# ariana-spalter/human-robot-gym

Hardware: AMD Instinct MI355X
Metric: env steps/sec (whole node), ReachHuman+shield 4096 envs (higher is better)
Workload: dtype f64

## Files before the change

human-robot-gym_amd/csrc/hrgym_device.h:

```cpp
#pragma once
#include <hip/hip_runtime.h>
#include <stdint.h>

#include "../../include/hrgym.h"
#include "../../include/hrgym_state.h"

#define NV HRG_NV
#define NARM HRG_NARM
#ifndef HRG_BOX
#define HRG_BOX 0
#endif
#ifndef HRG_LIFT
#define HRG_LIFT 0
#endif
#ifndef HRG_HANDOVER
#define HRG_HANDOVER 0
#endif
#ifndef HRG_STACK
#define HRG_STACK 0
#endif
#ifndef HRG_HULLS
#define HRG_HULLS 0
#endif
#ifndef HRG_HAMMER
// ... 96 lines not shown
#ifdef HRG_STAMPS
static __device__ unsigned long long g_stamps[32];
static __device__ unsigned long long g_stamps_slow[34];
static __device__ unsigned long long g_slow_thresh = ~0ull;
static __device__ unsigned long long g_envcyc[16384][3];
static __device__ unsigned long long g_envacc[16384][32];
__shared__ unsigned long long g_tbeg;
__shared__ unsigned long long g_acc[32];
__shared__ unsigned long long g_t0;
#define STAMP_NOW(var) do { __builtin_amdgcn_sched_barrier(0); asm volatile("s_memtime %0\n\ts_waitcnt lgkmcnt(0)" : "=s"(var) :: "memory"); __builtin_amdgcn_sched_barrier(0); } while (0)
#define STAMP_DECL
#define STAMP_INIT(lane) do { if ((lane) < 32) g_acc[lane] = 0; unsigned long long _t; STAMP_NOW(_t); g_t0 = _t; g_tbeg = _t; __syncthreads(); } while (0)
#define STAMP(k) do { unsigned long long _t; STAMP_NOW(_t); if (threadIdx.x == 0) { g_acc[k] += _t - g_t0; g_t0 = _t; } } while (0)
#define STAMP_FLUSH(lane)
#define COUNT(k, n) do { if (threadIdx.x == 0) g_acc[k] += (n); } while (0)
#define STAMP_FINAL(lane) do { __syncthreads(); if ((lane) < 32) atomicAdd(&g_stamps[lane], g_acc[lane]); { unsigned long long _te; STAMP_NOW(_te); if (_te - g_tbeg > g_slow_thresh) { if ((lane) < 32) atomicAdd(&g_stamps_slow[lane], g_acc[lane]); if ((lane) == 32) atomicAdd(&g_stamps_slow[32], 1ull); if ((lane) == 33) atomicAdd(&g_stamps_slow[33], _te - g_tbeg); } } if ((lane) < 32 && blockIdx.x < 16384) g_envacc[blockIdx.x][lane] = g_acc[lane]; if ((lane) == 0 && blockIdx.x < 16384) { unsigned long long _t; STAMP_NOW(_t); g_envcyc[blockIdx.x][0] = g_tbeg; g_envcyc[blockIdx.x][1] = _t; unsigned _hw, _xcc; asm volatile("s_getreg_b32 %0, hwreg(HW_REG_HW_ID)\n\ts_getreg_b32 %1, hwreg(HW_REG_XCC_ID)" : "=s"(_hw), "=s"(_xcc)); g_envcyc[blockIdx.x][2] = ((unsigned long long)_xcc << 32) | _hw; } } while (0)
#else
#define STAMP_DECL
#define STAMP_INIT(lane)
#define STAMP(k)
#define STAMP_FLUSH(lane)
#define COUNT(k, n)
#define STAMP_FINAL(lane)
#endif

struct DevModel {
  hrg_model_desc m;
  double Rbase[9];
  double Rq[NV][9];
  int32_t anc_mask[NV];
  int32_t hb_maxdepth;
  double sol_K, sol_Bd;
  double rcap_hl[HRG_NRCAP], hcap_hl[HRG_NHB];
  int32_t hb_njump;
  int32_t hb_jump[4][HRG_NHB];
  int32_t phase_mask;
  hrg_path brake_full;
  double brake_T, brake_ds;
  int32_t hc_n;
  struct alignas(32) HcRec { double th, v, al; int32_t kj, pad; } hc[HRG_NHCAP_MAX];
  int32_t n_self;
  struct alignas(32) SelfRec { int32_t ij, body_j; double inv_len2, bound, r_j; } self_rec[64];
  int32_t n_chk;
  int32_t chk_i[32], chk_j[32];
  hrg_clip_table clips;
  const double* pose_tab;
  const double* hull_dev;
  double hull_cen[HRG_NHULL][3];
  unsigned long long* mpr_fallback;
  double fric_D[NV + 1], fric_lim[NV + 1];
  double eul_hd[NV], eul_rhd[2];
  int32_t eul_fingers, eul_pad;
  double rcap_mid[HRG_NRCAP][3];
};

struct Contact {
  int32_t g1, g2, b1, b2;
  double dist, n[3], pos[3];
};

#define ROW_CON0 24
#define ROW_WELD0 (ROW_CON0 + 4 * NCON_DYN)
#if HRG_HAMMER
#define HROW_NFRIC 8
#define HROW_LIM0 9
#define HROW_NLIM 25
#define HROW_EQ0 27
#define HROW_CON0 36
#define HROW_NEQ 9
#define NROW 128
#elif HRG_STACK
#define SROW_WELD0 24
#define SROW_CON0 36
#define NROW HRG_NROW_STACK
#elif HRG_BOX && (HRG_HANDOVER || HRG_LIFT)
#define NROW (ROW_WELD0 + 6)
#else
#define NROW ROW_WELD0
#endif

struct GjkLds { double y[4][3], a[4][3], b[4][3], l[4], lam[4]; int ia[4], ib[4]; };
#define HRG_HULL_MPR (HRG_HULLS && (HRG_BOX || HRG_STACK || HRG_HAMMER))
#if HRG_HULL_MPR
struct MprLds { double v[5][3], a[5][3], b[5][3]; };
#endif
struct Lds {
  hrg_env_state st;
  double kR[NV][9], kp[NV][3], Sw[NV][3], Sv[NV][3], vw[NV][3], vv[NV][3];
  double M[NV * NV];
  double bias[NV], a0[NVS], Ma0[NVS], ctrl[NV], qacc[NVS], g[NVS], d[NVS];
#if HRG_BOX
  hrg_box_state bx;
  double bR[9];
  double bMr[9];
  double hand_q[4], hand_off[3];
  int palm_hit, palm_pad;
#if HRG_HANDOVER
  double hcap_keep[HRG_NHB][6];
#endif
#endif
  double act[NV];
#if HRG_POSE_TABLE
  double hyaw[9];
#endif
  int acc_has_collision, acc_collision_type, acc_failsafe, acc_pad;
#if HRG_HAMMER
// ... 592 lines not shown
  for (int k = 0; k < NV; k++) {
    const double akk = __shfl(a, k * 9, 64);
    if (!(akk > 0)) good = false;
    const double inv = rsqrt(akk), d = akk * inv;
    const double lik = __shfl(a, i * 8 + k, 64) * inv;
    const double ljk = __shfl(a, j * 8 + k, 64) * inv;
    if (j == k) { if (i == k) a = d; else if (i > k) a = lik; }
    else if (i > k && j > k) a -= lik * ljk;
  }
  *ok = good;
  return a;
}
template <bool ZEROS = false>
DI double chain_prefix(double x, int lane) {
  double y = ZEROS || lane < NARM ? x : 0.0;
  {
#pragma clang fp contract(off)
    y += dpp_f64<0x111>(y);
  }
  y += dpp_f64<0x112>(y);
  y += dpp_f64<0x114>(y);
  return lane < NARM ? y : y + x;
}
template <bool ZEROS = false>
DI double subtree_sum(double x, int lane) {
  double y = ZEROS || lane < NV ? x : 0.0;
  {
#pragma clang fp contract(off)
    y += dpp_f64<0x101>(y);
  }
  y += dpp_f64<0x102>(y);
  y += dpp_f64<0x104>(y);
  return lane < NARM ? y : x;
}
DI double uniform_f64(double v) {
  const long long b = __double_as_longlong(v);
  const int lo = __builtin_amdgcn_readfirstlane((int)(b & 0xffffffffLL));
  const int hi = __builtin_amdgcn_readfirstlane((int)(b >> 32));
  return __longlong_as_double(((long long)hi << 32) | (unsigned int)lo);
}
typedef __attribute__((address_space(3))) double LdsF64;
DI LdsF64* lds_lane_base(double* p) {
  unsigned a = (unsigned)(size_t)(LdsF64*)p;
  asm volatile("" : "+v"(a));
  return (LdsF64*)(size_t)a;
}
template <int K>
DI double lane_value(double v) {
  const long long b = __double_as_longlong(v);
  const int lo = __builtin_amdgcn_readlane((int)(b & 0xffffffffLL), K);
  const int hi = __builtin_amdgcn_readlane((int)(b >> 32), K);
  return __longlong_as_double(((long long)hi << 32) | (unsigned int)lo);
}
DI void cull_box(const double* cap, double rr, bool has, int lane, double* lo, double* hi) {
  const int g = lane >> 4;
  const long long flip = (long long)(g & 1) << 63;
  double e1 = -1e300, e2 = -1e300;
  if (has) {
    const int a = g >> 1;
    const double p1 = __longlong_as_double(__double_as_longlong(cap[a]) ^ flip), p2 = __longlong_as_double(__double_as_longlong(cap[3 + a]) ^ flip);
    e1 = max_f64(p1, p2) + rr;
    if (g < 2) {
      const double z1 = __longlong_as_double(__double_as_longlong(cap[2]) ^ flip), z2 = __longlong_as_double(__double_as_longlong(cap[5]) ^ flip);
      e2 = max_f64(z1, z2) + rr;
    }
  }
  e1 = row16_max(e1); e2 = row16_max(e2);
  hi[0] = lane_value<0>(e1); lo[0] = -lane_value<16>(e1); hi[1] = lane_value<32>(e1); lo[1] = -lane_value<48>(e1);
  hi[2] = lane_value<0>(e2); lo[2] = -lane_value<16>(e2);
}
#define HRG_PIVOT(v, K) lane_value<(K) * 9>(v)
template <int K>
DI void inv_pivot(double& a, int i, int j, bool& good) {
  const double akk = HRG_PIVOT(a, K);
  if (!(akk > 0)) good = false;
  const double pa = 1.0 / akk;
  const double aik = __shfl(a, i * 8 + K, 64);
  const double akj = __shfl(a, K * 8 + j, 64);
  if (i == K) a = j == K ? pa : akj * pa;
  else if (j == K) a = -aik * pa;
  else a -= aik * akj * pa;
}
DI double spd_inverse1(double a, int lane, bool* ok) {
  const int i = lane >> 3, j = lane & 7;
  bool good = true;
  inv_pivot<0>(a, i, j, good); inv_pivot<1>(a, i, j, good); inv_pivot<2>(a, i, j, good); inv_pivot<3>(a, i, j, good);
  inv_pivot<4>(a, i, j, good); inv_pivot<5>(a, i, j, good); inv_pivot<6>(a, i, j, good); inv_pivot<7>(a, i, j, good);
  *ok = good;
  return a;
}
DI double spd_inverse1_6(double a, int lane, bool* ok) {
  const int i = lane >> 3, j = lane & 7;
  bool good = true;
  inv_pivot<0>(a, i, j, good); inv_pivot<1>(a, i, j, good); inv_pivot<2>(a, i, j, good); inv_pivot<3>(a, i, j, good);
  inv_pivot<4>(a, i, j, good); inv_pivot<5>(a, i, j, good);
  *ok = good;
  return a;
}
template <int K>
DI void inv_pivot4(double* a, int i, int j, bool& good) {
#pragma unroll
  for (int q = 0; q < 4; q++) inv_pivot<K>(a[q], i, j, good);
}
DI void spd_inverse4(double* a, int lane, bool* ok) {
  const int i = lane >> 3, j = lane & 7;
  bool good = true;
  inv_pivot4<0>(a, i, j, good); inv_pivot4<1>(a, i, j, good); inv_pivot4<2>(a, i, j, good); inv_pivot4<3>(a, i, j, good);
  inv_pivot4<4>(a, i, j, good); inv_pivot4<5>(a, i, j, good);
  *ok = good;
}
template <int N> struct Tiles { double t[N][N]; };
DI double lane_value_dyn(double v, int k) {
  const long long b = __double_as_longlong(v);
  const int lo = __builtin_amdgcn_readlane((int)(b & 0xffffffffLL), k);
  const int hi = __builtin_amdgcn_readlane((int)(b >> 32), k);
  return __longlong_as_double(((long long)hi << 32) | (unsigned int)lo);
}
template <int N, int A, int A0>
DI void tiles_pivots(Tiles<N>& T, int i, int j, int np, bool& good) {
#pragma unroll 1
  for (int P = 0; P < np; P++) {
    const double akk = lane_value_dyn(T.t[A][A], P * 9);
// ... 44 lines not shown
```

human-robot-gym_amd/csrc/hrgym_hip.hip:

```cpp
#include <hip/hip_runtime.h>

#include <algorithm>
#include <cmath>
#include <cstdio>
#include <cstring>
#include <cstdlib>
#include <initializer_list>
#include <limits>
#include <memory>
#include <string>
#include <vector>

#include "hrgym_kernels.h"

template <class MD>
DI void impedance(const MD& m, double x0, double* imp) {
  const double d0 = m.solimp[0], dmax = m.solimp[1], width = m.solimp[2], mid = m.solimp[3], power = m.solimp[4];
  const double x = fabs(x0) / width;
  double y;
  if (x >= 1) y = 1;
  else if (x <= 0) y = 0;
  else if (x <= mid) { const double u = x / mid; y = u * u * mid; }
  else { const double u = (1 - x) / (1 - mid); y = 1 - u * u * (1 - mid); }
  (void)power;
// ... 2178 lines not shown
  const ModelPtr dm = uniform_model(dm_);
  Lds& L = g_L;
  const auto& m = dm->m;
  hrg_env_state& s = L.st;
      s.time = s.time + m.timestep;
  eef_update(dm_);
  const int hl = dm->clips.clip_holding_hand[clip_of(dm, gid, s.episode, s.anim_index)];
  const int site = hl ? m.site_lhand : m.site_rhand;
  wave_sync();
  if (lane < 3) {
    const double mp = s.human_site[site][lane] + L.hand_off[lane];
    L.bx.mocap_pos[lane] = mp;
    if (m.task == HRG_TASK_HANDOVER_R2H) L.bx.target[lane] = mp;
  }
  if (lane < 4) L.bx.mocap_quat[lane] = L.hand_q[lane];
  wave_sync();
  robot_chain_fk(dm_, lane, false);
  robot_dynamics_terms(dm_, lane);
  for (int k = lane; k < HRG_NHB * 6; k += 64) (&L.hcap[0][0])[k] = (&L.hcap_keep[0][0])[k];
  wave_sync();
}
#endif

#ifndef HRG_FAIR
#if HRG_HANDOVER || HRG_STACK || HRG_HAMMER
#define HRG_FAIR 0
#else
#define HRG_FAIR 2
#endif
#endif
#if HRG_FAIR
#ifndef FAIR_SCOPE
#define FAIR_SCOPE __HIP_MEMORY_SCOPE_WORKGROUP
#endif
DI int fair_key() {
  unsigned hw, xcc;
  asm volatile("s_getreg_b32 %0, hwreg(HW_REG_HW_ID)\n\ts_getreg_b32 %1, hwreg(HW_REG_XCC_ID)" : "=s"(hw), "=s"(xcc));
  const unsigned wave = hw & 0xf, simd = (hw >> 4) & 3, cu = (hw >> 8) & 0xf, sh = (hw >> 12) & 1, se = (hw >> 13) & 7;
  return (int)((((((xcc & 7) * 8 + se) * 2 + sh) * 16 + cu) * 4 + simd) * 8 + (wave & 7));
}
DI void fair_publish(int* g_fair, int lane, int progress) {
  const int key = fair_key();
  if (lane == 0) __hip_atomic_store(&g_fair[key], progress + 1, __ATOMIC_RELAXED, FAIR_SCOPE);
}
DI int fair_begin(int* g_fair, int lane, int progress) {
  const int key = fair_key(), base = key & ~7;
  if (lane == 0) __hip_atomic_store(&g_fair[key], progress + 1, __ATOMIC_RELAXED, FAIR_SCOPE);
  int v = 0;
  if (lane < 8) v = __hip_atomic_load(&g_fair[base + lane], __ATOMIC_RELAXED, FAIR_SCOPE);
  return v;
}
DI void fair_apply(int lane, int progress, int v, bool busy) {
  const int me = fair_key() & 7;
  const bool other = lane < 8 && lane != me && v > 0;
  int vmin = other ? v : 0x7fffffff, vmax = other ? v : 0;
#pragma unroll
  for (int o = 4; o > 0; o >>= 1) {
    const int a = __shfl_xor(vmin, o, 64), b = __shfl_xor(vmax, o, 64);
    vmin = a < vmin ? a : vmin; vmax = b > vmax ? b : vmax;
  }
  vmin = __builtin_amdgcn_readfirstlane(vmin); vmax = __builtin_amdgcn_readfirstlane(vmax);
  const int own = progress + 1;
  int pr;
  if (vmax == 0) pr = 0;
  else {
    pr = own < vmax ? (own <= vmin ? 3 : 2)
                    : (own > vmin ? 0 : 1);
  }
  if (busy && pr < 2) pr = 2;
  pr = __builtin_amdgcn_readfirstlane(pr);
  if (pr == 3) __builtin_amdgcn_s_setprio(3);
  else if (pr == 2) __builtin_amdgcn_s_setprio(2);
  else if (pr == 1) __builtin_amdgcn_s_setprio(1);
  else __builtin_amdgcn_s_setprio(0);
}
#endif

DI int cycle_body(const DevModel* __restrict__ dm_, int lane, int e, int64_t gid, int cyc, int busy, double* dbg_r, double* dbg_h, int32_t* dbg_nh, int32_t* fair) {
  (void)fair;
  asm volatile("" : "+v"(lane));
  const ModelPtr dm = uniform_model(dm_);
  Lds& L = g_L;
  const auto& m = dm->m;
  hrg_env_state& s = L.st;
  STAMP(0);
#define FAIR_P(k) cyc
#if HRG_FAIR
  int fair_v = fair_begin(fair, lane, FAIR_P(0));
  const bool fair_busy = __builtin_amdgcn_readfirstlane((busy || !s.is_safe) ? 1 : 0) != 0;
#elif !defined(HRG_NO_PRIO)
  if (__builtin_amdgcn_readfirstlane((busy || !s.is_safe) ? 1 : 0)) __builtin_amdgcn_s_setprio(3); else __builtin_amdgcn_s_setprio(0);
#endif
  if (cyc == 0) {
    if (lane < NARM) {
      const double scale = fabs(m.act_out_max - m.act_out_min) / fabs(m.act_in_max - m.act_in_min);
      const double otr = 0.5 * (m.act_out_max + m.act_out_min), itr = 0.5 * (m.act_in_max + m.act_in_min);
      const double a = clampd(L.act[lane], m.act_in_min, m.act_in_max);
      const double g = clampd(s.qpos[lane] + ((a - itr) * scale + otr), m.qpos_limits[0][lane], m.qpos_limits[1][lane]);
      s.goal_qpos[lane] = g;
      s.new_goal_q[lane] = g;
    }
    s.new_goal = 1;
    wave_sync();
  }
#ifdef HRG_STAMPS
  const int pm = dm->phase_mask;
#else
  constexpr int pm = 0xff;
#endif
  if (pm & 1) shield_step(dm_, lane, e, dbg_r, dbg_h, dbg_nh); else robot_chain_fk(dm_, lane, false);
  STAMP(1);
#if HRG_FAIR
  fair_apply(lane, FAIR_P(0), fair_v, fair_busy);
#endif
// ... 612 lines not shown
  quatmul(mq, q1, qa);
  human_fk_lanes(dm_, lane, mp, mq, fr + 7);
  constexpr int NP = 6 * HRG_NHB + 3 * HRG_NHJ;
  double* o = out + (size_t)k * 2 * NP;
  for (int j = lane; j < 6 * HRG_NHB; j += 64) o[j] = (&L.hcap[0][0])[j];
  for (int j = lane; j < 3 * HRG_NHJ; j += 64) o[6 * HRG_NHB + j] = (&s.human_site[0][0])[j];
  wave_sync();
  human_yaw_update();
  human_pose_from_table(dm, lane, f);
  for (int j = lane; j < 6 * HRG_NHB; j += 64) o[NP + j] = (&L.hcap[0][0])[j];
  for (int j = lane; j < 3 * HRG_NHJ; j += 64) o[NP + 6 * HRG_NHB + j] = (&s.human_site[0][0])[j];
}

__global__ __launch_bounds__(64) void hrg_wave_helpers_kernel(const double* __restrict__ in, unsigned long long mask, double* __restrict__ out) {
  const int lane = hrg_lane();
  const double x = in[lane];
  for (int k = 0; k < HRG_WAVE_NOUT; k++) out[64 * k + lane] = __builtin_nan("");
  if ((mask >> lane) & 1) {
    double* o = out + lane;
    o[64 * 0] = wave_sum(x);
    o[64 * 1] = row8_sum(x);
    o[64 * 2] = row16_max(x);
    o[64 * 3] = wave_max(x);
    o[64 * 4] = chain_prefix(x, lane);
    o[64 * 5] = subtree_sum(x, lane);
    o[64 * 6] = fsqrt(x);
    o[64 * 7] = dpp_f64<0xB1>(x);
    o[64 * 8] = dpp_f64<0x4E>(x);
    o[64 * 9] = dpp_f64<0x141>(x);
    o[64 * 10] = dpp_f64<0x140>(x);
    o[64 * 11] = dpp_f64<0x111>(x);
    o[64 * 12] = dpp_f64<0x112>(x);
    o[64 * 13] = dpp_f64<0x114>(x);
    o[64 * 14] = dpp_f64<0x101>(x);
    o[64 * 15] = dpp_f64<0x102>(x);
    o[64 * 16] = dpp_f64<0x104>(x);
    o[64 * 17] = dpp_f64_rows<0x142, 0xa>(x);
    o[64 * 18] = dpp_f64_rows<0x143, 0xc>(x);
    o[64 * 19] = __builtin_amdgcn_rsq(x);
    o[64 * 20] = chain_prefix<true>(lane < NARM ? x : 0.0, lane);
    o[64 * 21] = subtree_sum<true>(lane < NV ? x : 0.0, lane);
  }
}

__global__ __launch_bounds__(64) void hrg_cull_box_kernel(const double* __restrict__ in, int n, double* __restrict__ out) {
  const int lane = hrg_lane();
  const bool has = (lane & 15) < n;
  const int c = has ? lane & 15 : 0;
  double lo[3], hi[3];
  cull_box(in + 7 * c, in[7 * c + 6], has, lane, lo, hi);
  if (lane == 0) for (int a = 0; a < 3; a++) { out[a] = lo[a]; out[3 + a] = hi[a]; }
}

struct ModelConstants { double fric_D, fric_lim, fric_imp, eul_hd, eul_rhd, rcap_mid; int eul_fingers; };
static_assert(3 * HRG_NRCAP <= 64, "one lane per coordinate of a capsule's mid point");
DI ModelConstants model_constants(ModelPtr dm, int lane, double x0) {
  const auto& m = dm->m;
  ModelConstants c = {0, 0, 0, 0, 0, 0, 0};
  if (lane <= NV) {
    const bool nail = lane == NV;
    const int r = nail ? 0 : lane;
    const double floss = nail ? m.hm_nail_frictionloss : m.jnt_frictionloss[r], diag = nail ? m.hm_nail_invweight : m.dof_invweight0[r];
    if (floss > 0 && diag > 0) {
      c.fric_D = row_D(m, x0, diag, &c.fric_imp);
      c.fric_lim = floss / c.fric_D;
    }
  }
  {
    const double h = m.timestep;
    const double hd6 = h * m.jnt_damping[NARM], hd7 = h * m.jnt_damping[NARM + 1];
    const bool fingers = hd6 > 0 && hd7 > 0;
    c.eul_fingers = fingers;
    if (lane < NV) c.eul_hd = h * m.jnt_damping[lane];
    if (lane < 2) c.eul_rhd = fingers ? 1.0 / (lane ? hd7 : hd6) : 0.0;
  }
  if (lane < 3 * HRG_NRCAP) {
    const int cc = lane / 3, a = lane - 3 * cc;
    c.rcap_mid = 0.5 * (m.rcap_p1[cc][a] + m.rcap_p2[cc][a]);
  }
  return c;
}
__global__ __launch_bounds__(64) void hrg_model_constants_kernel(DevModel* __restrict__ dmw) {
  const ModelPtr dm = uniform_model(dmw);
  const int lane = hrg_lane();
  const ModelConstants c = model_constants(dm, lane, 0.0);
  if (lane <= NV) { dmw->fric_D[lane] = c.fric_D; dmw->fric_lim[lane] = c.fric_lim; }
  if (lane < NV) dmw->eul_hd[lane] = c.eul_hd;
  if (lane < 2) dmw->eul_rhd[lane] = c.eul_rhd;
  if (lane == 0) dmw->eul_fingers = c.eul_fingers;
  if (lane < 3 * HRG_NRCAP) (&dmw->rcap_mid[0][0])[lane] = c.rcap_mid;
}
__global__ __launch_bounds__(64) void hrg_model_constants_tap_kernel(const DevModel* __restrict__ dm_, double x0, double* __restrict__ out) {
  const ModelPtr dm = uniform_model(dm_);
  const int lane = hrg_lane();
  const ModelConstants c = model_constants(dm, lane, x0);
  double* st = out, *re = out + HRG_MC_DIM;
  if (lane <= NV) {
    const bool fr = dm_->fric_D[lane] != 0;
    st[HRG_MC_FRIC_D + lane] = dm_->fric_D[lane]; re[HRG_MC_FRIC_D + lane] = c.fric_D;
    st[HRG_MC_FRIC_LIM + lane] = dm_->fric_lim[lane]; re[HRG_MC_FRIC_LIM + lane] = c.fric_lim;
    st[HRG_MC_FRIC_IMP + lane] = fr ? dm->m.solimp[0] : 0.0; re[HRG_MC_FRIC_IMP + lane] = c.fric_imp;
  }
  if (lane < NV) { st[HRG_MC_EUL_HD + lane] = dm_->eul_hd[lane]; re[HRG_MC_EUL_HD + lane] = c.eul_hd; }
  if (lane < 2) { st[HRG_MC_EUL_RHD + lane] = dm_->eul_rhd[lane]; re[HRG_MC_EUL_RHD + lane] = c.eul_rhd; }
  if (lane == 0) { st[HRG_MC_EUL_FINGERS] = dm_->eul_fingers; re[HRG_MC_EUL_FINGERS] = c.eul_fingers; }
  if (lane < 3 * HRG_NRCAP) { st[HRG_MC_RCAP_MID + lane] = (&dm_->rcap_mid[0][0])[lane]; re[HRG_MC_RCAP_MID + lane] = c.rcap_mid; }
}
#endif

__global__ __launch_bounds__(64) void HRG_SYM(hrg_chain_fk_kernel)(const DevModel* __restrict__ dm_, const double* __restrict__ q, int n, int shield_on, double* __restrict__ out) {
  const int lane = hrg_lane(), k = (int)blockIdx.x;
  if (k >= n) return;
  Lds& L = g_L;
  const double* qk = q + (size_t)k * 3 * NARM;
  if (lane < NARM) { L.cq[lane] = qk[lane]; L.qe[lane] = qk[NARM + lane]; }
  if (lane < NV) L.st.qpos[lane] = lane < NARM ? qk[2 * NARM + lane] : 0.0;
  wave_sync();
  robot_chain_fk(dm_, lane, shield_on != 0);
  double* o = out + (size_t)k * HRG_CFK_DIM;
  for (int j = lane; j < 9 * NV; j += 64) o[HRG_CFK_KR + j] = (&L.kR[0][0])[j];
  if (lane < 3 * NV) o[HRG_CFK_KP + lane] = (&L.kp[0][0])[lane];
  for (int j = lane; j < 2 * HRG_NSHIELD_RCAP * 6; j += 64) o[HRG_CFK_SCAP + j] = shield_on ? (&L.scap[0][0][0])[j] : 0.0;
}

__global__ __launch_bounds__(64) void HRG_SYM(hrg_self_pairs_kernel)(const DevModel* __restrict__ dm_, const double* __restrict__ q, int n, double* __restrict__ out) {
  const int lane = hrg_lane(), k = (int)blockIdx.x;
  if (k >= n) return;
  const ModelPtr dm = uniform_model(dm_);
  Lds& L = g_L;
  if (lane < NV) L.st.qpos[lane] = lane < NARM ? q[(size_t)k * NARM + lane] : 0.0;
  wave_sync();
  robot_chain_fk(dm_, lane, false);
  wave_sync();
  robot_capsules_world(dm, lane);
  wave_sync();
  double* o = out + (size_t)k * HRG_SP_DIM;
  if (lane < 6 * HRG_NRCAP) o[HRG_SP_CAPS + lane] = (&L.rcapw[0][0])[lane];
  const bool valid = lane < dm->n_self;
  const SelfPair sp = self_pair(dm, valid ? lane : 0);
  const bool near = valid && self_near(sp);
  double* op = o + HRG_SP_PAIRS + HRG_SP_PDIM * lane;
  for (int a = 0; a < HRG_SP_PDIM; a++) op[a] = 0.0;
  if (valid) { op[0] = sp.i; op[1] = sp.j; op[2] = near ? 1.0 : 0.0; }
// ... 168 lines not shown
```

human-robot-gym_amd/csrc/hrgym_host_batch.h:

```cpp

struct TaskTraits;
struct hrg_batch {
  int device = 0;
  int32_t n_envs = 0;
  int64_t env_id0 = 0;
  DeviceMem mem;
  DevModel* d_model = nullptr;
  double* d_frames = nullptr;
  double* d_pose = nullptr;
  size_t pose_bytes = 0;
  double* d_hull = nullptr;
  bool hulls = false;
  unsigned long long* d_mpr_fallback = nullptr;
  hrg_env_state* d_states = nullptr;
  double* d_rcaps = nullptr;
  double* d_hcaps = nullptr;
  int32_t* d_nh = nullptr;
  float* d_scratch_obs = nullptr;
  hrg_box_state* d_boxes = nullptr;
  hrg_stack_state* d_stacks = nullptr;
  hrg_hammer_state* d_hammers = nullptr;
  int32_t* d_order = nullptr;
  int32_t parity = 0;
  const TaskTraits* traits = nullptr;
// ... 141 lines not shown
    if (desc->scap_body[c] != (c < NARM ? c : NARM - 1)) return fail(HRG_ERR_INVALID, "shield capsule c must sit on link c (gripper on link 6)");
  if (desc->n_bodypart > HRG_NBODYPART_MAX || desc->n_extremity > HRG_NEXTREMITY_MAX) return fail(HRG_ERR_INVALID, "too many body parts");
  const TaskTraits* const t = task_traits(desc->task);
  if (!t) return fail(HRG_ERR_UNSUPPORTED, "unknown task");
  if (desc->task == HRG_TASK_STACKING) {
    if (!(desc->box_inertia[0] == desc->box_inertia[1] && desc->box_inertia[1] == desc->box_inertia[2]))
      return fail(HRG_ERR_UNSUPPORTED, "CollaborativeStackingCart: the HIP stepper stacks cubes (object_full_size with three equal edges)");
    for (int c = 0; c < clips->n_clips; c++) {
      const int32_t* kf = clips->clip_stack_keyframes[c];
      if (!(kf[0] >= 0 && kf[0] <= kf[1] && kf[1] <= kf[2] && kf[2] <= kf[3] && kf[3] <= kf[4] && clips->clip_n_loop[c] >= 0 && clips->clip_n_loop[c] <= HRG_MAX_LOOP &&
            clips->clip_n_loop2[c] >= 0 && clips->clip_n_loop2[c] <= HRG_MAX_LOOP))
        return fail(HRG_ERR_INVALID, "CollaborativeStackingCart: every clip needs five ascending keyframes and at most 4 loop sines per waiting phase in its info");
    }
  }
  if (desc->task == HRG_TASK_LIFTING && !(desc->min_balance > -1 && desc->min_balance < 1)) return fail(HRG_ERR_INVALID, "CollaborativeLiftingCart: min_balance must lie in (-1, 1)");
  if (HRG_IS_HANDOVER(desc->task))
    for (int c = 0; c < clips->n_clips; c++)
      if (!(clips->clip_n_loop2[c] >= 0 && clips->clip_n_loop2[c] <= HRG_MAX_LOOP)) return fail(HRG_ERR_INVALID, "HumanRobotHandoverCart: at most 4 loop sines per stage");
  if (desc->task == HRG_TASK_INSPECTION || HRG_IS_HANDOVER(desc->task))
    for (int c = 0; c < clips->n_clips; c++)
      if (!(clips->clip_n_loop[c] >= 0 && clips->clip_n_loop[c] <= HRG_MAX_LOOP && clips->clip_keyframes[c][0] >= 0 && clips->clip_keyframes[c][0] <= clips->clip_keyframes[c][1]))
        return fail(HRG_ERR_INVALID, "HumanObjectInspectionCart: every clip needs keyframes (k0 <= k1) and at most 4 loop sines in its info");
  if (desc->ik_enabled && !(desc->ik_max_iter >= 1 && desc->ik_max_iter <= 1000 && desc->ik_damping > 0 && desc->ik_action_limit > 0 && desc->ik_residual_threshold >= 0))
    return fail(HRG_ERR_INVALID, "ik: need 1 <= max_iter <= 1000, damping > 0, action_limit > 0, residual_threshold >= 0");
  if (desc->task == HRG_TASK_HAMMERING) {
    if (!(desc->hm_board_mass > 0 && desc->hm_hammer_mass > 0 && desc->hm_nail_mass > 0 && desc->hm_nail_range > 0 && desc->hm_nail_invweight > 0 && desc->n_obj_placements > 0 &&
          desc->hm_board_inertia[0] > 0 && desc->hm_board_inertia[1] > 0 && desc->hm_board_inertia[2] > 0 && desc->hm_hammer_inertia[0] > 0 && desc->hm_hammer_inertia[1] > 0 &&
          desc->hm_hammer_inertia[2] > 0))
      return fail(HRG_ERR_INVALID, "CollaborativeHammeringCart needs positive board / hammer / nail masses and inertias, a nail range and n_obj_placements > 0");
    for (int c = 0; c < clips->n_clips; c++)
      if (!(clips->clip_keyframes[c][0] >= 0 && clips->clip_keyframes[c][0] <= clips->clip_keyframes[c][1] && clips->clip_n_loop[c] >= 0 && clips->clip_n_loop[c] <= HRG_MAX_LOOP))
        return fail(HRG_ERR_INVALID, "CollaborativeHammeringCart: every clip needs two ascending keyframes and at most 4 loop sines in its info");
  } else
  if (t->objs != HRG_OBJ_NONE && !(desc->box_half[0] > 0 && desc->box_half[1] > 0 && desc->box_half[2] > 0 && desc->box_mass > 0 && desc->box_inertia[0] > 0 && desc->box_inertia[1] > 0 &&
                                     desc->box_inertia[2] > 0 && desc->box_inertia_mean > 0 && desc->box_invweight_rot > 0 && desc->n_targets > 0 && desc->n_obj_placements > 0))
    return fail(HRG_ERR_INVALID, "PickPlaceHumanCart needs box_half, box_mass, box_inertia, n_targets, n_obj_placements > 0");
  int maxd = 0;
  for (int i = 0; i < HRG_NHB; i++) maxd = desc->hb_depth[i] > maxd ? desc->hb_depth[i] : maxd;
  if (maxd + 1 > 16) return fail(HRG_ERR_INVALID, "human tree deeper than 15");
  int n_in_pos = 0;
  for (int k = 0; k < desc->n_bodypart; k++) {
    if (desc->bp_joint[k][0] < 0 || desc->bp_joint[k][0] >= HRG_NHJ || desc->bp_joint[k][1] < 0 || desc->bp_joint[k][1] >= HRG_NHJ) return fail(HRG_ERR_INVALID, "body part joint outside the human's sites");
    n_in_pos += desc->bp_in_pos[k] ? 1 : 0;
  }
  for (int k = 0; k < desc->n_extremity; k++)
    if (desc->ext_joint[k] < 0 || desc->ext_joint[k] >= HRG_NHJ) return fail(HRG_ERR_INVALID, "extremity joint outside the human's sites");
  if (2 * desc->n_bodypart + desc->n_extremity + n_in_pos > HRG_NHCAP_MAX) return fail(HRG_ERR_INVALID, "more than 64 human reach capsules");
  int64_t tot = 0;
  for (int c = 0; c < clips->n_clips; c++) {
    if (clips->clip_len[c] < 1 || clips->clip_offset[c] != tot) return fail(HRG_ERR_INVALID, "clip table must be densely packed");
    tot += clips->clip_len[c];
  }
  if (tot != clips->total_frames) return fail(HRG_ERR_INVALID, "clip table total_frames mismatch");
  if (desc->robot_hulls) {
    if (!g_variants.v[t->family][1].step)
      return fail(HRG_ERR_UNSUPPORTED, "robot_hulls: no hull variant of the step kernel for this task");
    if (!desc->hull_verts || desc->hull_off[0] != 0) return fail(HRG_ERR_INVALID, "robot_hulls: hull_verts / hull_off missing");
    for (int h = 0; h < HRG_NHULL; h++)
      if (!(desc->hull_off[h + 1] > desc->hull_off[h] + 3 && desc->hull_off[h + 1] <= 1000000)) return fail(HRG_ERR_INVALID, "robot_hulls: every hull needs at least four vertices");
  }
  return HRG_OK;
}

static void batch_fill_model(const hrg_model_desc* desc, const hrg_clip_table* clips, DevModel* hm) {
  memset(hm, 0, sizeof *hm);
  hm->m = *desc;
  mat_from_quat(hm->Rbase, desc->base_quat);
  for (int i = 0; i < NV; i++) {
    mat_from_quat(hm->Rq[i], desc->body_quat[i]);
    int mask = 0;
    for (int k = i; k >= 0; k = desc->body_parent[k]) mask |= 1 << k;
    hm->anc_mask[i] = mask;
  }
  int maxd = 0;
  for (int i = 0; i < HRG_NHB; i++) maxd = desc->hb_depth[i] > maxd ? desc->hb_depth[i] : maxd;
  hm->hb_maxdepth = maxd;
  {
    double tc = desc->solref[0];
    const double dr = desc->solref[1], dmax = desc->solimp[1];
    if (tc < 2 * desc->timestep) tc = 2 * desc->timestep;
    hm->sol_K = 1.0 / (dmax * dmax * tc * tc * dr * dr);
    hm->sol_Bd = 2.0 / (dmax * tc);
  }
  for (int c = 0; c < HRG_NRCAP; c++) {
    double d2 = 0;
    for (int a = 0; a < 3; a++) d2 += (desc->rcap_p2[c][a] - desc->rcap_p1[c][a]) * (desc->rcap_p2[c][a] - desc->rcap_p1[c][a]);
    hm->rcap_hl[c] = 0.5 * sqrt(d2);
  }
  for (int c = 0; c < HRG_NHB; c++) {
    double d2 = 0;
    for (int a = 0; a < 3; a++) d2 += (desc->hcap_p2[c][a] - desc->hcap_p1[c][a]) * (desc->hcap_p2[c][a] - desc->hcap_p1[c][a]);
    hm->hcap_hl[c] = 0.5 * sqrt(d2);
  }
  for (int i = 0; i < HRG_NHB; i++) hm->hb_jump[0][i] = desc->hb_parent[i];
  for (int s = 1; s < 4; s++)
    for (int i = 0; i < HRG_NHB; i++) { const int a = hm->hb_jump[s - 1][i]; hm->hb_jump[s][i] = a < 0 ? -1 : hm->hb_jump[s - 1][a]; }
  hm->hb_njump = 0;
  while ((1 << hm->hb_njump) < maxd + 1) hm->hb_njump++;
  int n = 0;
  auto hc_set = [&](int n, int kind, int j1, int j2, double th, double v, double al) { hm->hc[n].th = th; hm->hc[n].v = v; hm->hc[n].al = al; hm->hc[n].kj = kind | (j1 << 8) | (j2 << 16); hm->hc[n].pad = 0; };
  for (int k = 0; k < desc->n_bodypart; k++, n++) hc_set(n, 0, desc->bp_joint[k][0], desc->bp_joint[k][1], desc->bp_thickness[k], desc->bp_vmax[k], desc->bp_amax[k]);
  for (int k = 0; k < desc->n_bodypart; k++, n++) hc_set(n, 1, desc->bp_joint[k][0], desc->bp_joint[k][1], desc->bp_thickness[k], desc->bp_vmax[k], 0.0);
  for (int k = 0; k < desc->n_extremity; k++, n++) hc_set(n, 2, desc->ext_joint[k], desc->ext_joint[k], desc->ext_thickness[k], desc->ext_vmax[k], desc->ext_length[k]);
  for (int k = 0; k < desc->n_bodypart; k++)
    if (desc->bp_in_pos[k]) hc_set(n++, 3, desc->bp_joint[k][0], desc->bp_joint[k][1], desc->bp_thickness[k], desc->bp_vmax[k], 0.0);
  hm->hc_n = n;
  int ns = 0;
  for (int i = 0; i < HRG_NRCAP; i++)
    for (int j = i + 1; j < HRG_NRCAP; j++)
      if ((desc->rcap_selfmask[i] >> j) & 1u) {
        double len2[2];
        for (int e = 0; e < 2; e++) {
          const int c = e ? j : i;
          len2[e] = 0;
          for (int a = 0; a < 3; a++) len2[e] += (desc->rcap_p2[c][a] - desc->rcap_p1[c][a]) * (desc->rcap_p2[c][a] - desc->rcap_p1[c][a]);
        }
        const bool seg_j = len2[1] > len2[0];
        const int s = seg_j ? j : i, o = seg_j ? i : j;
        DevModel::SelfRec& r = hm->self_rec[ns++];
        r.ij = i | (j << 8) | (s << 16) | (o << 24);
        r.body_j = desc->rcap_body[j];
        r.inv_len2 = len2[seg_j] <= 1e-12 ? 0.0 : 1.0 / len2[seg_j];
        r.bound = hm->rcap_hl[o] + desc->rcap_r[i] + desc->rcap_r[j] + 1e-9;
        r.r_j = desc->rcap_r[j];
      }
  hm->n_self = ns;
  int nc = 0;
  for (int i = 0; i < 8; i++)
    for (int j = i + 1; j < 8; j++)
      if (((desc->chk_selfmask[i] >> j) & 1u) && nc < 32) { hm->chk_i[nc] = i; hm->chk_j[nc] = j; nc++; }
  hm->n_chk = nc;
  hm->phase_mask = 0xff;
  {
    double se, ve, ae;
    path_plan(&hm->brake_full, 0.0, 1.0, 0.0, desc->failsafe_sdot, desc->path_amax, desc->path_jmax);
    hm->brake_T = path_total(&hm->brake_full);
    path_eval(&hm->brake_full, hm->brake_T, desc->failsafe_sdot, &se, &ve, &ae);
    hm->brake_ds = se;
  }
#ifdef HRG_STAMPS
  if (const char* pm = getenv("HRG_PHASE_MASK")) hm->phase_mask = atoi(pm);
#endif
  hm->clips = *clips;
  if (desc->robot_hulls) hull_centroids(desc->hull_verts, desc->hull_off, hm->hull_cen);
}

static int batch_upload(hrg_batch* b, const hrg_model_desc* desc, const hrg_clip_table* clips, DevModel* hm) {
  DeviceMem& m = b->mem;
  const size_t frames = (size_t)clips->total_frames;
  bool ok = m.upload(b->d_frames, clips->frames, HRG_FRAME_DIM * frames);
  if (ok && b->traits->pose_table) {
    b->pose_bytes = sizeof(double) * HRG_POSE_DIM * frames;
    ok = m.zeros(b->d_pose, HRG_POSE_DIM * frames);
  }
  if (ok && desc->robot_hulls)
    ok = m.upload(b->d_hull, desc->hull_verts, 3 * (size_t)desc->hull_off[HRG_NHULL]) && m.zeros(b->d_mpr_fallback, 1);
  hm->clips.frames = b->d_frames;
  hm->pose_tab = b->d_pose;
  hm->hull_dev = b->d_hull;
  hm->mpr_fallback = b->d_mpr_fallback;
  if (!ok || !m.upload(b->d_model, hm, 1)) return nomem("batch", m);
  hipLaunchKernelGGL(hrg_model_constants_kernel, dim3(1), dim3(64), 0, 0, b->d_model);
  HIPCHK(hipGetLastError());
  HIPCHK(hipDeviceSynchronize());
  if (b->d_pose) {
    hipLaunchKernelGGL(hrg_pose_table_kernel, dim3((unsigned)clips->total_frames), dim3(64), 0, 0, b->d_model, b->d_pose);
    HIPCHK(hipGetLastError());
    HIPCHK(hipDeviceSynchronize());
  }
  return HRG_OK;
}

static int batch_env_arrays(hrg_batch* b) {
  const size_t n = (size_t)b->n_envs;
  std::vector<hrg_env_state> init(n);
  memset(init.data(), 0, sizeof(hrg_env_state) * n);
  for (auto& s : init) s.episode = -1;
  std::vector<int32_t> ord(2 * n + 4, 0);
  for (size_t e = 0; e < n; e++) ord[e] = ord[n + e] = (int32_t)e;
// ... 421 lines not shown
```

human-robot-gym_amd/csrc/hrgym_kernels.h:

```cpp
#pragma once
#include "hrgym_device.h"
#if HRG_HULLS
#include "hrgym_hull.h"
#endif

DI double chain_dot(double a0, double a1, double a2, double b0, double b1, double b2) {
#pragma clang fp contract(off)
  return __builtin_fma(a2, b2, __builtin_fma(a0, b0, a1 * b1));
}
DI double chain_acc(double a0, double a1, double a2, double b0, double b1, double b2) {
  return __builtin_fma(a2, b2, __builtin_fma(a1, b1, __builtin_fma(a0, b0, 0.0)));
}
DI void robot_chain_fk(const DevModel* __restrict__ dm_, int lane, bool shield_on) {
  const ModelPtr dm = uniform_model(dm_);
  Lds& L = g_L;
  if (lane < 3 * NARM && (lane >= 2 * NARM || shield_on)) {
    const int cfg = lane / NARM, i = lane - NARM * cfg;
    const double q = cfg == 0 ? L.cq[i] : (cfg == 1 ? L.qe[i] : L.st.qpos[i]);
    double sn, cs;
    sincos_small(q, &sn, &cs);
    LdsF64* o = lds_lane_base(&L.rc[0][0] + 2 * lane);
    o[0] = sn; o[1] = cs;
  }
  wave_sync();
// ... 1209 lines not shown
        if (ok && dist < 0) {
          hit = true;
          v3set(c.n, 0, 0, 1);
          v3set(c.pos, p[0], p[1], z0 + 0.5 * dist);
          c.g1 = pl ? GEOM_FLOOR : GEOM_TABLE; c.g2 = GEOM_BOX + g; c.b1 = -1; c.b2 = BODY_BOX + fb; c.dist = dist;
        }
      }
      const uint64_t mask = __ballot(hit);
      if (hit) {
        const int slot = base + __popcll(mask & lt);
        if (slot < NCON_DYN) L.con[slot] = c;
        if (slot < HRG_NCON_MAX) { L.st.con_pairs[slot][0] = c.g1; L.st.con_pairs[slot][1] = c.g2; }
      }
      base += __popcll(mask);
    } else {
      int nc = 0;
      BBContact bc[4];
      int ga = HRG_HG_HEAD, gb = HRG_HG_NAIL;
      if (lane < 4) {
        ga = (lane & 1) ? HRG_HG_HANDLE : HRG_HG_HEAD; gb = lane < 2 ? HRG_HG_NAIL : HRG_HG_BOARD;
        const double ha[3] = {m.hm_geom_half[ga][0], m.hm_geom_half[ga][1], m.hm_geom_half[ga][2]}, hb[3] = {m.hm_geom_half[gb][0], m.hm_geom_half[gb][1], m.hm_geom_half[gb][2]};
        double d[3], d2 = 0;
        v3sub(d, L.gc[ga], L.gc[gb]);
        for (int a = 0; a < 3; a++) {
          const double la = fabs(L.gR[0][a] * d[0] + L.gR[0][3 + a] * d[1] + L.gR[0][6 + a] * d[2]) - hb[a];
          if (la > 0) d2 += la * la;
        }
        const double ra = fsqrt(ha[0] * ha[0] + ha[1] * ha[1] + ha[2] * ha[2]) + 1e-9;
        static_assert(40 * (NVS + 1) + 4 * BB_WORK <= (4 * NCON_DYN + HROW_NEQ) * (NVS + 1), "box_box2 workspace of the four box pairs");
#if HRG_HULLS
        static_assert(__builtin_offsetof(Lds, gjk) + sizeof(GjkLds) <= __builtin_offsetof(Lds, Jc) + sizeof(L.Jc[0]) * 40 &&
                      __builtin_offsetof(Lds, mpr) + sizeof(MprLds) <= __builtin_offsetof(Lds, Jc) + sizeof(L.Jc[0]) * 40, "the GJK simplex / MPR portal and the box_box2 workspace alias");
#endif
        if (!(d2 > ra * ra)) nc = box_box2(L.gc[ga], L.gR[1], ha, L.gc[gb], L.gR[0], hb, bc, &L.Jc[40][0] + BB_WORK * lane);
      }
      int pre = 0, tot = 0;
      for (int q = 0; q < 4; q++) { const int nq = __shfl(nc, q, 64); if (q < lane) pre += nq; tot += nq; }
      for (int q = 0; q < nc; q++) {
        const int slot = base + pre + q;
        c.g1 = GEOM_BOX + ga; c.g2 = GEOM_BOX + gb; c.b1 = BODY_BOX + HRG_HM_HAMMER; c.b2 = BODY_BOX + (gb == HRG_HG_NAIL ? HRG_HM_NAIL : HRG_HM_BOARD); c.dist = bc[q].dist;
        v3cpy(c.n, bc[q].n); v3cpy(c.pos, bc[q].pos);
        if (slot < NCON_DYN) L.con[slot] = c;
        if (slot < HRG_NCON_MAX) { L.st.con_pairs[slot][0] = c.g1; L.st.con_pairs[slot][1] = c.g2; }
      }
      base += tot;
    }
  }
  hm.gripped = f0 && f1;
  *base_io = base;
}
#endif
DI void robot_capsules_world(ModelPtr dm, int lane) {
  Lds& L = g_L;
  const auto& m = dm->m;
  if (lane < HRG_NRCAP) {
    const int c = lane, b = m.rcap_body[c];
    double R[9], p[3], t[3];
    if (b < 0) { for (int a = 0; a < 9; a++) R[a] = dm->Rbase[a]; v3cpy(p, m.base_pos); }
    else { for (int a = 0; a < 9; a++) R[a] = L.kR[b][a]; v3cpy(p, L.kp[b]); }
    m3mulv(t, R, m.rcap_p1[c]); v3add(&L.rcapw[c][0], p, t);
    m3mulv(t, R, m.rcap_p2[c]); v3add(&L.rcapw[c][3], p, t);
  }
}
struct SelfPair { int i, j, s, o, body_j; double inv_len2, bound, r_j; };
DI SelfPair self_pair(ModelPtr dm, int k) {
  const struct { int ij, body_j; double inv_len2, bound, r_j; } rec = {dm->self_rec[k].ij, dm->self_rec[k].body_j, dm->self_rec[k].inv_len2, dm->self_rec[k].bound, dm->self_rec[k].r_j};
  return SelfPair{rec.ij & 0xff, (rec.ij >> 8) & 0xff, (rec.ij >> 16) & 0xff, rec.ij >> 24, rec.body_j, rec.inv_len2, rec.bound, rec.r_j};
}
DI bool self_near(const SelfPair& sp) {
  const Lds& L = g_L;
  const double *p = &L.rcapw[sp.s][0], *q = &L.rcapw[sp.o][0];
  double d[3], w[3], e[3];
  for (int a = 0; a < 3; a++) { d[a] = p[3 + a] - p[a]; w[a] = 0.5 * (q[a] + q[3 + a]) - p[a]; }
  const double t = fmin(fmax(v3dot(w, d) * sp.inv_len2, 0.0), 1.0);
  for (int a = 0; a < 3; a++) e[a] = w[a] - t * d[a];
  return v3dot(e, e) <= sp.bound * sp.bound;
}
template <class Model>
DI bool capsule_pair_contact(const Model& m, int i, const double* a1, const double* a2, double r2, double margin, int g2, Contact& c) {
  const Lds& L = g_L;
  double c1[3], c2[3], d[3];
  const double d2 = seg_seg(&L.rcapw[i][0], &L.rcapw[i][3], a1, a2, c1, c2), dd = fsqrt(d2), dist = dd - m.rcap_r[i] - r2;
  if (!(dist < margin)) return false;
  v3sub(d, c2, c1);
  if (dd > 1e-12) v3scl(c.n, d, 1.0 / dd);
  v3madd(c.pos, c1, c.n, m.rcap_r[i] + 0.5 * dist);
  c.g1 = i; c.g2 = g2; c.b1 = m.rcap_body[i]; c.dist = dist;
  return true;
}
PH_COLLIDE void collide(const DevModel* __restrict__ dm_, int lane, int* ncon_out) {
  const ModelPtr dm = uniform_model(dm_);
  Lds& L = g_L;
  const auto& m = dm->m;
  robot_capsules_world(dm, lane);
  wave_sync();
  int n_hnear;
  {
    static_assert(HRG_NRCAP <= 16 && HRG_NSHIELD_RCAP <= 16, "cull_box: one DPP row of capsules");
    double lo[3], hi[3];
    {
      const bool has = (lane & 15) < HRG_NRCAP;
      const int rc = has ? lane & 15 : 0;
      cull_box(&L.rcapw[rc][0], m.rcap_r[rc] + m.contact_margin_human + 1e-9, has, lane, lo, hi);
    }
    double d2 = 0;
    const int hb = lane < HRG_NHB ? lane : 0;
    for (int a = 0; a < 3; a++) {
      const double c = 0.5 * (L.hcap[hb][a] + L.hcap[hb][3 + a]);
      const double e = c < lo[a] ? lo[a] - c : (c > hi[a] ? c - hi[a] : 0.0);
      d2 += e * e;
    }
    const double rad = dm->hcap_hl[hb] + m.hcap_r[hb] + 1e-9;
    const bool hn = lane < HRG_NHB && d2 <= rad * rad;
    const uint64_t hmask = __ballot(hn);
    n_hnear = __popcll(hmask);
    if (hn) L.hnear[__popcll(hmask & ((1ull << lane) - 1))] = lane;
    if (n_hnear) wave_sync();
  }
  int base = 0;
  const uint64_t lt = lane == 0 ? 0ull : (~0ull >> (64 - lane));
  const int n_hpairs = HRG_NRCAP * n_hnear, n_hrounds = (n_hpairs + 63) >> 6;
  const float inv_hnear = n_hnear ? 1.0f / (float)n_hnear : 0.0f;
#pragma unroll 1
  for (int round = 0; round < 2 + n_hrounds; round++) {
    bool hit = false;
    Contact c;
    c.g1 = c.g2 = c.b1 = c.b2 = 0; c.dist = 0; v3set(c.n, 0, 0, 1); v3set(c.pos, 0, 0, 0);
    if (round <= n_hrounds) {
      int i = 0, g2 = 0;
      double r2 = 0, margin = 0, hl2 = 0;
      const double *a1, *a2;
      bool valid, near = false;
      if (round == 0) {
        valid = lane < dm->n_self;
        const SelfPair sp = self_pair(dm, valid ? lane : 0);
        i = sp.i;
        g2 = sp.j; a1 = &L.rcapw[sp.j][0]; a2 = &L.rcapw[sp.j][3]; r2 = sp.r_j;
        c.b2 = sp.body_j;
        near = valid && self_near(sp);
      } else {
        const int q = (round - 1) * 64 + lane;
        valid = q < n_hpairs;
        i = valid ? (int)(((float)q + 0.5f) * inv_hnear) : 0;
        const int hb = valid ? L.hnear[q - i * n_hnear] : 0;
        g2 = GEOM_HUMAN0 + hb; a1 = &L.hcap[hb][0]; a2 = &L.hcap[hb][3]; r2 = m.hcap_r[hb]; hl2 = dm->hcap_hl[hb];
        margin = m.contact_margin_human;
        c.b2 = -2;
        if (valid) {
          double ca[3], cb[3], dc[3];
          for (int a = 0; a < 3; a++) { ca[a] = 0.5 * (L.rcapw[i][a] + L.rcapw[i][3 + a]); cb[a] = 0.5 * (a1[a] + a2[a]); }
          v3sub(dc, ca, cb);
          const double reach = dm->rcap_hl[i] + hl2 + m.rcap_r[i] + r2 + margin + 1e-9;
          near = v3dot(dc, dc) <= reach * reach;
        }
      }
      if (__any(near) && valid && near) hit = capsule_pair_contact(m, i, a1, a2, r2, margin, g2, c);
    } else if (lane < 4 * HRG_NRCAP) {
      const int pl = lane / (2 * HRG_NRCAP), i = (lane % (2 * HRG_NRCAP)) >> 1, en = lane & 1;
      if (m.rcap_body[i] >= 0) {
        const double* p = &L.rcapw[i][3 * en];
        const double z0 = pl ? m.floor_z : m.table_top_z, dist = p[2] - m.rcap_r[i] - z0;
        bool ok = true;
        if (pl == 0) ok = fabs(p[0] - m.table_center[0]) <= m.table_half[0] && fabs(p[1] - m.table_center[1]) <= m.table_half[1] && p[2] > z0 - 0.025;
        if (ok && dist < 0) {
          hit = true;
          v3set(c.n, 0, 0, -1);
          v3set(c.pos, p[0], p[1], z0 + 0.5 * dist);
          c.g1 = i; c.g2 = pl ? GEOM_FLOOR : GEOM_TABLE; c.b1 = m.rcap_body[i]; c.b2 = -1; c.dist = dist;
        }
      }
    }
#if HRG_HULLS
    if (m.robot_hulls) {
      uint64_t todo = __ballot(hit && c.g1 < HRG_NHULL && c.g2 >= GEOM_HUMAN0);
      int last_plane = -1;
      while (todo) {
        const int src = __ffsll((unsigned long long)todo) - 1;
        todo &= todo - 1;
        const int g1 = __builtin_amdgcn_readlane(c.g1, src), g2 = __builtin_amdgcn_readlane(c.g2, src);
        const int lb = m.rcap_body[g1];
        const HullRef H = {dm_->hull_dev + 3 * m.hull_off[g1], m.hull_off[g1 + 1] - m.hull_off[g1], lb < 0 ? dm_->Rbase : L.kR[lb], lb < 0 ? dm_->m.base_pos : L.kp[lb]};
        if (g2 < GEOM_TABLE) {
          const int hb = g2 - GEOM_HUMAN0;
          double wa[3], wb[3];
          const double dh = gjk_hull_segment_wave(H, &L.hcap[hb][0], &L.hcap[hb][3], wa, wb, (m.hcap_r[hb] + m.contact_margin_human) * (1.0 + 1e-9));
          if (dh > 1e-9 && lane == src) {
            const double dist = dh - m.hcap_r[hb];
            if (!(dist < m.contact_margin_human)) hit = false;
            else {
              for (int a = 0; a < 3; a++) { c.n[a] = (wb[a] - wa[a]) / dh; c.pos[a] = wa[a] + c.n[a] * (0.5 * dist); }
              c.dist = dist;
            }
// ... 280 lines not shown
```

Before: 5.015 million.

## Skip collision rounds when no self, human, or ground contact is possible

Adds an early-out to collide: self-pair proximity is computed once as a ballot, and cull_box gains a z-minimum reduction over moving capsules. When no self pair is near, no human capsule is near, and all capsules sit above table and floor, the whole contact-round loop is skipped. Capsule world-position computation is spread across one lane per endpoint coordinate, using precomputed per-lane records and base-fixed capsules precomputed in model constants. fair_apply also swaps shuffle reductions for readlane loops. The z-bound test must stay conservative, or real ground contacts would be missed.

New measurement: 5.080 million (median of 6 runs). 1.3% higher.

```diff
diff --git a/human-robot-gym_amd/csrc/hrgym_device.h b/human-robot-gym_amd/csrc/hrgym_device.h
--- a/human-robot-gym_amd/csrc/hrgym_device.h
+++ b/human-robot-gym_amd/csrc/hrgym_device.h
@@ -172,6 +172,7 @@
   double eul_hd[NV], eul_rhd[2];
   int32_t eul_fingers, eul_pad;
   double rcap_mid[HRG_NRCAP][3];
+  struct alignas(32) RcapLane { double v[3]; int32_t k, pad; } rcap_lane[6 * HRG_NRCAP];
 };
 
 struct Contact {
@@ -870,7 +871,8 @@
   const int hi = __builtin_amdgcn_readlane((int)(b >> 32), K);
   return __longlong_as_double(((long long)hi << 32) | (unsigned int)lo);
 }
-DI void cull_box(const double* cap, double rr, bool has, int lane, double* lo, double* hi) {
+template <bool ZMIN = false>
+DI void cull_box(const double* cap, double rr, bool has, int lane, double* lo, double* hi, double rz = 0, bool hasz = false, double* zmin = nullptr) {
   const int g = lane >> 4;
   const long long flip = (long long)(g & 1) << 63;
   double e1 = -1e300, e2 = -1e300;
@@ -878,7 +880,12 @@
     const int a = g >> 1;
     const double p1 = __longlong_as_double(__double_as_longlong(cap[a]) ^ flip), p2 = __longlong_as_double(__double_as_longlong(cap[3 + a]) ^ flip);
     e1 = max_f64(p1, p2) + rr;
-    if (g < 2) {
+    if (ZMIN) {
+      const long long flipz = (long long)((g | (g >> 1)) & 1) << 63;
+      const double z1 = __longlong_as_double(__double_as_longlong(cap[2]) ^ flipz), z2 = __longlong_as_double(__double_as_longlong(cap[5]) ^ flipz);
+      const double ez = max_f64(z1, z2) + (g < 2 ? rr : rz);
+      if (g < 2 || (g == 2 && hasz)) e2 = ez;
+    } else if (g < 2) {
       const double z1 = __longlong_as_double(__double_as_longlong(cap[2]) ^ flip), z2 = __longlong_as_double(__double_as_longlong(cap[5]) ^ flip);
       e2 = max_f64(z1, z2) + rr;
     }
@@ -886,6 +893,7 @@
   e1 = row16_max(e1); e2 = row16_max(e2);
   hi[0] = lane_value<0>(e1); lo[0] = -lane_value<16>(e1); hi[1] = lane_value<32>(e1); lo[1] = -lane_value<48>(e1);
   hi[2] = lane_value<0>(e2); lo[2] = -lane_value<16>(e2);
+  if (ZMIN) *zmin = -lane_value<32>(e2);
 }
 #define HRG_PIVOT(v, K) lane_value<(K) * 9>(v)
 template <int K>
diff --git a/human-robot-gym_amd/csrc/hrgym_hip.hip b/human-robot-gym_amd/csrc/hrgym_hip.hip
--- a/human-robot-gym_amd/csrc/hrgym_hip.hip
+++ b/human-robot-gym_amd/csrc/hrgym_hip.hip
@@ -2254,14 +2254,13 @@
 }
 DI void fair_apply(int lane, int progress, int v, bool busy) {
   const int me = fair_key() & 7;
-  const bool other = lane < 8 && lane != me && v > 0;
-  int vmin = other ? v : 0x7fffffff, vmax = other ? v : 0;
-#pragma unroll
-  for (int o = 4; o > 0; o >>= 1) {
-    const int a = __shfl_xor(vmin, o, 64), b = __shfl_xor(vmax, o, 64);
-    vmin = a < vmin ? a : vmin; vmax = b > vmax ? b : vmax;
-  }
-  vmin = __builtin_amdgcn_readfirstlane(vmin); vmax = __builtin_amdgcn_readfirstlane(vmax);
+  (void)lane;
+  int vmin = 0x7fffffff, vmax = 0;
+#pragma unroll
+  for (int k = 0; k < 8; k++) {
+    const int vk = __builtin_amdgcn_readlane(v, k);
+    if (k != me && vk > 0) { vmin = vk < vmin ? vk : vmin; vmax = vk > vmax ? vk : vmax; }
+  }
   const int own = progress + 1;
   int pr;
   if (vmax == 0) pr = 0;
@@ -2980,11 +2979,17 @@
   if (lane == 0) for (int a = 0; a < 3; a++) { out[a] = lo[a]; out[3 + a] = hi[a]; }
 }
 
-struct ModelConstants { double fric_D, fric_lim, fric_imp, eul_hd, eul_rhd, rcap_mid; int eul_fingers; };
+struct ModelConstants { double fric_D, fric_lim, fric_imp, eul_hd, eul_rhd, rcap_mid, rcap_base; int eul_fingers; };
 static_assert(3 * HRG_NRCAP <= 64, "one lane per coordinate of a capsule's mid point");
+static_assert(6 * HRG_NRCAP <= 64, "one lane per coordinate of a capsule's end points");
 DI ModelConstants model_constants(ModelPtr dm, int lane, double x0) {
   const auto& m = dm->m;
-  ModelConstants c = {0, 0, 0, 0, 0, 0, 0};
+  ModelConstants c = {0, 0, 0, 0, 0, 0, 0, 0};
+  if (lane < 6 * HRG_NRCAP) {
+    const int cc = lane / 6, e = (lane - 6 * cc) / 3, a = lane - 6 * cc - 3 * e;
+    const auto* v = e ? m.rcap_p2[cc] : m.rcap_p1[cc];
+    c.rcap_base = m.base_pos[a] + chain_dot(dm->Rbase[3 * a], dm->Rbase[3 * a + 1], dm->Rbase[3 * a + 2], v[0], v[1], v[2]);
+  }
   if (lane <= NV) {
     const bool nail = lane == NV;
     const int r = nail ? 0 : lane;
@@ -3017,6 +3022,7 @@
   if (lane < 2) dmw->eul_rhd[lane] = c.eul_rhd;
   if (lane == 0) dmw->eul_fingers = c.eul_fingers;
   if (lane < 3 * HRG_NRCAP) (&dmw->rcap_mid[0][0])[lane] = c.rcap_mid;
+  if (lane < 6 * HRG_NRCAP && dm->m.rcap_body[lane / 6] < 0) dmw->rcap_lane[lane].v[0] = c.rcap_base;
 }
 __global__ __launch_bounds__(64) void hrg_model_constants_tap_kernel(const DevModel* __restrict__ dm_, double x0, double* __restrict__ out) {
   const ModelPtr dm = uniform_model(dm_);
diff --git a/human-robot-gym_amd/csrc/hrgym_host_batch.h b/human-robot-gym_amd/csrc/hrgym_host_batch.h
--- a/human-robot-gym_amd/csrc/hrgym_host_batch.h
+++ b/human-robot-gym_amd/csrc/hrgym_host_batch.h
@@ -217,6 +217,8 @@
     tot += clips->clip_len[c];
   }
   if (tot != clips->total_frames) return fail(HRG_ERR_INVALID, "clip table total_frames mismatch");
+  for (int c = 0; c < HRG_NRCAP; c++)
+    if (desc->rcap_body[c] < -1 || desc->rcap_body[c] >= NV) return fail(HRG_ERR_INVALID, "rcap_body: a robot capsule rides on the base (-1) or on a body of the tree");
   if (desc->robot_hulls) {
     if (!g_variants.v[t->family][1].step)
       return fail(HRG_ERR_UNSUPPORTED, "robot_hulls: no hull variant of the step kernel for this task");
@@ -290,6 +292,12 @@
         r.r_j = desc->rcap_r[j];
       }
   hm->n_self = ns;
+  for (int l = 0; l < 6 * HRG_NRCAP; l++) {
+    const int c = l / 6, e = (l % 6) / 3, a = l % 3, bd = desc->rcap_body[c];
+    DevModel::RcapLane& r = hm->rcap_lane[l];
+    for (int q = 0; q < 3; q++) r.v[q] = e ? desc->rcap_p2[c][q] : desc->rcap_p1[c][q];
+    r.k = bd < 0 ? -1 : 3 * bd + a;
+  }
   int nc = 0;
   for (int i = 0; i < 8; i++)
     for (int j = i + 1; j < 8; j++)
diff --git a/human-robot-gym_amd/csrc/hrgym_kernels.h b/human-robot-gym_amd/csrc/hrgym_kernels.h
--- a/human-robot-gym_amd/csrc/hrgym_kernels.h
+++ b/human-robot-gym_amd/csrc/hrgym_kernels.h
@@ -1285,14 +1285,12 @@
 #endif
 DI void robot_capsules_world(ModelPtr dm, int lane) {
   Lds& L = g_L;
-  const auto& m = dm->m;
-  if (lane < HRG_NRCAP) {
-    const int c = lane, b = m.rcap_body[c];
-    double R[9], p[3], t[3];
-    if (b < 0) { for (int a = 0; a < 9; a++) R[a] = dm->Rbase[a]; v3cpy(p, m.base_pos); }
-    else { for (int a = 0; a < 9; a++) R[a] = L.kR[b][a]; v3cpy(p, L.kp[b]); }
-    m3mulv(t, R, m.rcap_p1[c]); v3add(&L.rcapw[c][0], p, t);
-    m3mulv(t, R, m.rcap_p2[c]); v3add(&L.rcapw[c][3], p, t);
+  if (lane < 6 * HRG_NRCAP) {
+    const struct { double v0, v1, v2; int k; } rec = {dm->rcap_lane[lane].v[0], dm->rcap_lane[lane].v[1], dm->rcap_lane[lane].v[2], dm->rcap_lane[lane].k};
+    const int k = rec.k < 0 ? 0 : rec.k;
+    const double* R = &L.kR[0][0] + 3 * k;
+    const double w = (&L.kp[0][0])[k] + chain_dot(R[0], R[1], R[2], rec.v0, rec.v1, rec.v2);
+    (&L.rcapw[0][0])[lane] = rec.k < 0 ? rec.v0 : w;
   }
 }
 struct SelfPair { int i, j, s, o, body_j; double inv_len2, bound, r_j; };
@@ -1328,13 +1326,15 @@
   robot_capsules_world(dm, lane);
   wave_sync();
   int n_hnear;
+  double zmin;
   {
     static_assert(HRG_NRCAP <= 16 && HRG_NSHIELD_RCAP <= 16, "cull_box: one DPP row of capsules");
     double lo[3], hi[3];
     {
       const bool has = (lane & 15) < HRG_NRCAP;
       const int rc = has ? lane & 15 : 0;
-      cull_box(&L.rcapw[rc][0], m.rcap_r[rc] + m.contact_margin_human + 1e-9, has, lane, lo, hi);
+      const double rz = m.rcap_r[rc];
+      cull_box<true>(&L.rcapw[rc][0], rz + m.contact_margin_human + 1e-9, has, lane, lo, hi, rz, m.rcap_body[rc] >= 0, &zmin);
     }
     double d2 = 0;
     const int hb = lane < HRG_NHB ? lane : 0;
@@ -1354,8 +1354,17 @@
   const uint64_t lt = lane == 0 ? 0ull : (~0ull >> (64 - lane));
   const int n_hpairs = HRG_NRCAP * n_hnear, n_hrounds = (n_hpairs + 63) >> 6;
   const float inv_hnear = n_hnear ? 1.0f / (float)n_hnear : 0.0f;
+  uint64_t self_mask;
+  {
+    const bool valid = lane < dm->n_self;
+    self_mask = __ballot(valid && self_near(self_pair(dm, valid ? lane : 0)));
+  }
+  const bool rounds = self_mask != 0 || n_hnear != 0 || !(zmin >= m.table_top_z && zmin >= m.floor_z);
+#if !HRG_HAMMER
+  if (!rounds) COUNT(30, 1);
+#endif
 #pragma unroll 1
-  for (int round = 0; round < 2 + n_hrounds; round++) {
+  for (int round = 0; rounds && round < 2 + n_hrounds; round++) {
     bool hit = false;
     Contact c;
     c.g1 = c.g2 = c.b1 = c.b2 = 0; c.dist = 0; v3set(c.n, 0, 0, 1); v3set(c.pos, 0, 0, 0);
@@ -1370,7 +1379,7 @@
         i = sp.i;
         g2 = sp.j; a1 = &L.rcapw[sp.j][0]; a2 = &L.rcapw[sp.j][3]; r2 = sp.r_j;
         c.b2 = sp.body_j;
-        near = valid && self_near(sp);
+        near = (self_mask >> lane) & 1;
       } else {
         const int q = (round - 1) * 64 + lane;
         valid = q < n_hpairs;
```
